# kasirershahartau/tissue_image_processing

Measured on AMD Instinct MI355X. Metric: frames/sec end-to-end (2048^2, z=30), higher is better.
Workload: dtype f32(f16x3)

## Files before the change

include/tissue_hip.h:

```cpp
#ifndef TISSUE_HIP_H
#define TISSUE_HIP_H

#include <stddef.h>
#include <stdint.h>

#ifdef __cplusplus
extern "C" {
#endif

#define TIP_API __attribute__((visibility("default")))

typedef enum {
    TIP_OK = 0,
    TIP_ERR_HIP = -1,
    TIP_ERR_ARG = -2,
    TIP_ERR_NOMEM = -3,
    TIP_ERR_INDEX = -4,
    TIP_ERR_UNSUPPORTED = -5,
    TIP_ERR_OVERFLOW = -6
} tip_status;

TIP_API int tip_init(int device);
TIP_API int tip_shutdown(void);
TIP_API int tip_last_error(char *buf, size_t n);
// ... 62 lines not shown
    const void *in0, *in1;
    int c0, c1, h, w, planes;
    const void *weights;
    int ntaps, dy[9], dx[9];
    int cout;
    const float *bias, *scale, *shift;
    void *out;
    int out_h, out_w, sy, sx, oy, ox;
    void *pool_out;
    const float *head_w, *head_b;
    float *head_out;
    int format;
    float acc_scale;
} tip_unet_conv_desc;
TIP_API int tip_unet_conv_dev(const tip_unet_conv_desc *d, void *stream);
TIP_API int tip_unet_conv_first_dev(const float *in, int h, int w, const float *wgt, const float *bias, const float *scale,
                                    const float *shift, void *out, int planes, int format, void *stream);
TIP_API int tip_unet_pool2_dev(const void *in, int h, int w, int ch, int planes, int format, void *out, void *stream);
TIP_API int tip_unet_head_dev(const void *in, long npix, const float *wgt, const float *bias, float *out, int planes, int format,
                              int logits, void *stream);
TIP_API int tip_unet_prepare_f64_dev(const double *img, int c, int a, int b, long cstride, long sa, long sb, int kind, float *out,
                                     int ap, int bp, void *stream);
TIP_API int tip_unet_tail_dev(const void *p, int dtype, long ld, int y, int x, double thr, int32_t *labels, double *hc,
                              int32_t *flags_host);

TIP_API int tip_draw_cell_types_u8(const uint8_t *types, long n, int must_mask, int lack_mask, const double *pos_rgb,
                                   const double *neg_rgb, double *out3);
TIP_API int tip_draw_tracking_i32(const int32_t *track, long n, const double *cycle18, double *out3);
TIP_API int tip_draw_disks_f64(int y, int x, int n, const double *cy, const double *cx, double radius, const double *rgb, double *out3);
TIP_API int tip_draw_lines_f64(int y, int x, int n, const int32_t *ends, const double *rgb, double *out3);
// ... 66 lines not shown
```

tissue_image_processing_amd/_unet_hip.py:

```python
import ctypes
import os
import threading

import numpy as np

from . import _lib

_MODES = {
    "f16x3": (2, 1, 3, "7.2e-7"),
    "bf16x3": (2, 0, 3, "1.6e-5"),
    "bf16x6": (3, 0, 6, "9e-8"),
}
_F16_ACT_SCALE = 16.0


class _ConvDesc(ctypes.Structure):
    _fields_ = [("in0", ctypes.c_void_p), ("in1", ctypes.c_void_p), ("c0", ctypes.c_int), ("c1", ctypes.c_int), ("h", ctypes.c_int),
                ("w", ctypes.c_int), ("planes", ctypes.c_int), ("weights", ctypes.c_void_p), ("ntaps", ctypes.c_int),
                ("dy", ctypes.c_int * 9), ("dx", ctypes.c_int * 9), ("cout", ctypes.c_int), ("bias", ctypes.c_void_p),
                ("scale", ctypes.c_void_p), ("shift", ctypes.c_void_p), ("out", ctypes.c_void_p), ("out_h", ctypes.c_int),
                ("out_w", ctypes.c_int), ("sy", ctypes.c_int), ("sx", ctypes.c_int), ("oy", ctypes.c_int), ("ox", ctypes.c_int),
                ("pool_out", ctypes.c_void_p), ("head_w", ctypes.c_void_p), ("head_b", ctypes.c_void_p), ("head_out", ctypes.c_void_p),
                ("format", ctypes.c_int), ("acc_scale", ctypes.c_float)]

# ... 151 lines not shown
        return out

    def first(h, w):
        out = buf(h, w, 128)
        timed("first %dx%d 2->128" % (h, w), 2.0 * h * w * 18 * 128,
              lambda: _lib.check(lib.tip_unet_conv_first_dev(D(x), h, w, D(hw["first"]), D(hw["f:d0.c1.b"]), D(hw["f:d0.b1.s"]),
                                                             D(hw["f:d0.b1.t"]), D(out), planes, fmt, stream)))
        return out

    def double(blk, src, skip, h, w, pooled=None, head=None):
        a = first(h, w) if src is None else conv3(blk + ".c1", blk + ".b1", src, skip, h, w)
        return conv3(blk + ".c2", blk + ".b2", a, None, h, w, pooled=pooled, head=head)

    def conv_t(name, src, h, w):
        up = buf(2 * h, 2 * w, hw[name + ".00"][0].shape[2] * 128)
        for py in (0, 1):
            for px in (0, 1):
                cls = "%s.%d%d" % (name, py, px)
                launch_conv(cls, _conv_desc(hw[cls], planes, fmt, src, None, h, w, hw["f:" + name + ".b"], out=up, out_h=2 * h, out_w=2 * w,
                                            stride=2, oy=py, ox=px))
        return up

    with torch.no_grad():
        skips, cur, h, w = [], None, H, W
        for i in range(3):
            pooled = buf(h // 2, w // 2, net.filters[i])
            skips.append(double("d%d" % i, cur, None, h, w, pooled=pooled))
            cur, h, w = pooled, h // 2, w // 2
        cur = double("mid", cur, None, h, w)
        for i in range(3):
            up = conv_t("u%d.t" % i, cur, h, w)
            h, w = 2 * h, 2 * w
            probs = None
            if i == 2 and not logits and not os.environ.get("TISSUE_HIP_UNET_SEPARATE_HEAD"):
                probs = torch.empty((1, 2, H, W), dtype=torch.float32, device=x.device)
# ... 9 lines not shown
```

tissue_image_processing_amd/csrc/tip_core.hip:

```cpp
#include "tip_internal.h"
#include <algorithm>
#include <cmath>
#include <cstdlib>
#include <map>
#include <mutex>

namespace tip {

static thread_local Ctx *g_ctx = nullptr;
static thread_local int g_requested_device = 0;

static int ctx_create(int device)
{
    Ctx *c = new Ctx();
    c->device = device;
    hipError_t e = hipSetDevice(device);
    if (e != hipSuccess) {
        c->err = std::string("hipSetDevice failed: ") + hipGetErrorString(e);
        g_ctx = c;
        return TIP_ERR_HIP;
    }
    {
        const char *pr = getenv("TIP_STREAM_PRIORITY");
        int lo = 0, hi = 0;
// ... 126 lines not shown
    }
    else if (n == "TIP_WS_OPEN") pair(t.ws_open_a, t.ws_open_b, def.ws_open_a, def.ws_open_b);
    else if (n == "TIP_WS_NO_SKIP") flag(t.ws_no_skip, 0);
    else if (n == "TIP_WS_DEBUG") flag(t.ws_debug, 0);
    else if (n == "TIP_WS_NO_ENDGAME") flag(t.ws_no_endgame, 0);
    else if (n == "TIP_WS_NO_WIDE") flag(t.ws_no_wide, 0);
    else if (n == "TIP_PROJECT_GENERIC") flag(t.project_generic, 0);
    else if (n == "TIP_PROJECT_UNFUSED_PREBLUR") flag(t.project_unfused_preblur, 0);
    else if (n == "TIP_PROJECT_UNFUSED_MASK") flag(t.project_unfused_mask, 0);
    else if (n == "TIP_PROJECT_EXACT_SCORE") flag(t.project_exact_score, 0);
    else if (n == "TIP_PROJECT_DEBUG") flag(t.project_debug, 0);
    else if (n == "TIP_UNET_TILE8") num(t.unet_tile8, def.unet_tile8);
    else if (n == "TIP_UF_ONE_LEVEL") flag(t.uf_one_level, 0);
    else if (n == "TIP_UNET_SPB") num(t.unet_spb, def.unet_spb);
    else if (n == "TIP_UNET_XCD_MAP") flag(t.unet_xcd_map, 1);
    else if (n == "TIP_UNET_TAIL_UNFUSED") flag(t.unet_tail_unfused, 0);
    else if (n == "TIP_MB_SMALL") num(t.mb_small, def.mb_small);
    else if (n == "TIP_MB_BATCH") num(t.mb_batch, def.mb_batch);
    else return false;
    return true;
}

const char *const TUNING_NAMES[] = {"TIP_WS_TIES", "TIP_WS_OPEN", "TIP_WS_NO_SKIP", "TIP_WS_DEBUG", "TIP_WS_NO_ENDGAME", "TIP_WS_NO_WIDE",
                                    "TIP_PROJECT_GENERIC", "TIP_PROJECT_UNFUSED_PREBLUR", "TIP_PROJECT_UNFUSED_MASK",
                                    "TIP_PROJECT_EXACT_SCORE", "TIP_PROJECT_DEBUG", "TIP_UNET_TILE8", "TIP_UNET_TAIL_UNFUSED", "TIP_UNET_XCD_MAP", "TIP_UNET_SPB", "TIP_UF_ONE_LEVEL", "TIP_MB_SMALL", "TIP_MB_BATCH"};

void tuning_from_env()
{
    for (const char *name : TUNING_NAMES)
        if (const char *e = getenv(name)) tuning_assign(g_tuning, name, e);
}
}

const Tuning &tuning()
{
    std::call_once(g_tuning_once, tuning_from_env);
    return g_tuning;
}

int make_taps(Taps &t, const double *w, int n)
// ... 225 lines not shown
```

tissue_image_processing_amd/csrc/tip_internal.h:

```cpp
#pragma once
#include <hip/hip_runtime.h>
#include <cstdarg>
#include <cstdint>
#include <cstdio>
#include <cstring>
#include <string>
#include <vector>
#include "../../include/tissue_hip.h"

namespace tip {

struct ProfRec { const char *name; hipEvent_t e0, e1; };

struct Ctx {
    int device = -1;
    hipStream_t stream = nullptr;
    std::string err;
    struct Block { void *p; size_t bytes; bool used; };
    std::vector<Block> pool;
    int last_ws_labels = 0;
    long last_ws_other = 0;
    hipEvent_t edge_event = nullptr;
    void *prep_ws = nullptr;
    void *pin_buf = nullptr;
// ... 20 lines not shown
};

void prof_begin(const char *name);
void prof_end();

struct Tuning {
    int ws_ties = 1;
    int ws_open_a = -1, ws_open_b = -1;
    int ws_no_skip = 0;
    int ws_debug = 0;
    int ws_no_endgame = 0, ws_no_wide = 0;
    int project_generic = 0, project_unfused_preblur = 0, project_unfused_mask = 0;
    int project_exact_score = 0, project_debug = 0;
    int unet_tail_unfused = 0;
    int unet_xcd_map = 1;
    int unet_spb = 3;
    int uf_one_level = 0;
    int mb_small = -1;
    int mb_batch = -1;
    int unet_tile8 = -1;
};
const Tuning &tuning();

#define TIP_HIP(call)                                                                             \
    do {                                                                                          \
        hipError_t e__ = (call);                                                                  \
        if (e__ != hipSuccess)                                                                    \
            return tip::fail(TIP_ERR_HIP, "%s failed: %s (%s:%d)", #call, hipGetErrorString(e__), \
                             __FILE__, __LINE__);                                                 \
    } while (0)
// ... 32 lines not shown
```

tissue_image_processing_amd/csrc/tip_unet.hip:

```cpp
#include "tip_internal.h"
#include "tip_unet_conv.h"
#include <algorithm>
#include <atomic>

namespace tip {

__global__ void __launch_bounds__(256) k_bias_relu_affine_f32(float *__restrict__ x, const float *__restrict__ bias,
                                                              const float *__restrict__ scale, const float *__restrict__ shift,
                                                              long n4, int C)
{
    const long i = (long)blockIdx.x * blockDim.x + threadIdx.x;
    if (i >= n4) return;
    float4 v = reinterpret_cast<float4 *>(x)[i];
    const int c = (int)((i * 4) % C);
    const float4 b = *reinterpret_cast<const float4 *>(bias + c);
    const float4 s = *reinterpret_cast<const float4 *>(scale + c);
    const float4 t = *reinterpret_cast<const float4 *>(shift + c);
    v.x += b.x; v.y += b.y; v.z += b.z; v.w += b.w;
    v.x = v.x > 0.f ? v.x : 0.f; v.y = v.y > 0.f ? v.y : 0.f; v.z = v.z > 0.f ? v.z : 0.f; v.w = v.w > 0.f ? v.w : 0.f;
    v.x = v.x * s.x + t.x; v.y = v.y * s.y + t.y; v.z = v.z * s.z + t.z; v.w = v.w * s.w + t.w;
    reinterpret_cast<float4 *>(x)[i] = v;
}

int rankfilter2d_dev(const void *in, void *out, int dtype, int Y, int X, int ky, int kx, int fp, int border, int is_max);
// ... 345 lines not shown
    for (int shift = 56; shift >= 0; shift -= 8) {
        hipLaunchKernelGGL(k_prep_hist, hgrid, dim3(256), 0, s, img, cstride, n, st, shift);
        hipLaunchKernelGGL(k_prep_pick, dim3(1), dim3(64), 0, s, st, c, shift);
    }
    hipLaunchKernelGGL(k_prep_next, hgrid, dim3(256), 0, s, img, cstride, n, st);
    hipLaunchKernelGGL(k_prep_finish, dim3(1), dim3(64), 0, s, st, c, g1, g99, kind);
    if (ap != a || bp != b) TIP_HIP(hipMemsetAsync(out, 0, (size_t)c * ap * bp * sizeof(float), s));
    const dim3 ngrid((unsigned)cdiv(a, 32), (unsigned)cdiv(b, 32), (unsigned)c);
    if (a_contig)
        hipLaunchKernelGGL(k_prep_normalize<true>, ngrid, dim3(256), 0, s, img, cstride, sa, sb, a, b, (const PrepState *)st, kind == 1 ? 1 : 0, out, ap, bp, ap - a, bp - b);
    else
        hipLaunchKernelGGL(k_prep_normalize<false>, ngrid, dim3(256), 0, s, img, cstride, sa, sb, a, b, (const PrepState *)st, kind == 1 ? 1 : 0, out, ap, bp, ap - a, bp - b);
    return unet_launch_check("unet_prepare");
}

int tip_unet_conv_dev(const tip_unet_conv_desc *d, void *stream)
{
    Ctx &c = ctx();
    if (!c.stream) return TIP_ERR_HIP;
    if (!d || !d->in0 || !d->weights || !d->bias || (!d->out && !d->head_out)) return fail(TIP_ERR_ARG, "tip_unet_conv_dev: null pointer");
    if (d->planes != 2 && d->planes != 3) return fail(TIP_ERR_ARG, "tip_unet_conv_dev: planes must be 2 or 3");
    if (d->format != 0 && d->format != 1) return fail(TIP_ERR_ARG, "tip_unet_conv_dev: format is 0 (bf16 pieces) or 1 (fp16 pieces)");
    if (d->format == 1 && (d->planes != 2 || !(d->acc_scale > 0.f))) return fail(TIP_ERR_ARG, "tip_unet_conv_dev: fp16 pieces come in two planes with a positive acc_scale");
    if (d->h < 8 || d->w < UC_TW || d->h % 8 || d->w % UC_TW)
        return fail(TIP_ERR_UNSUPPORTED, "tip_unet_conv_dev: the grid %dx%d is not a multiple of the 8x%d pixel tile", d->h, d->w, UC_TW);
    if (d->c0 < UC_KC || d->c0 % UC_KC || d->c1 < 0 || d->c1 % UC_KC || (d->c1 > 0 && !d->in1) || d->cout < UC_BN || d->cout % UC_BN)
        return fail(TIP_ERR_UNSUPPORTED, "tip_unet_conv_dev: channels (%d + %d -> %d) must be multiples of %d / %d", d->c0, d->c1, d->cout, UC_KC, UC_BN);
    if (d->ntaps < 1 || d->ntaps > 9 || d->sy < 1 || d->sx < 1 || d->oy < 0 || d->ox < 0 ||
        (d->h - 1) * d->sy + d->oy >= d->out_h || (d->w - 1) * d->sx + d->ox >= d->out_w)
        return fail(TIP_ERR_ARG, "tip_unet_conv_dev: bad taps / output mapping");
    if ((d->scale == nullptr) != (d->shift == nullptr)) return fail(TIP_ERR_ARG, "tip_unet_conv_dev: scale and shift come together");
    if (18L * d->w * (d->c0 > d->c1 ? d->c0 : d->c1) * 2 >= (1L << 32) - 65536)
        return fail(TIP_ERR_UNSUPPORTED, "tip_unet_conv_dev: 18 rows of %d pixels x %d channels exceed the 4 GB a buffer resource addresses",
                    d->w, d->c0 > d->c1 ? d->c0 : d->c1);
    ConvParams p;
    p.in0 = (const uint16_t *)d->in0; p.in1 = (const uint16_t *)(d->c1 > 0 ? d->in1 : d->in0);
    p.c0 = d->c0; p.c1 = d->c1; p.H = d->h; p.W = d->w;
    p.w = (const uint16_t *)d->weights; p.ntaps = d->ntaps;
    for (int t = 0; t < 9; ++t) {
        p.dy[t] = t < d->ntaps ? d->dy[t] : 0; p.dx[t] = t < d->ntaps ? d->dx[t] : 0;
        if (p.dy[t] < -1 || p.dy[t] > 1 || p.dx[t] < -1 || p.dx[t] > 1) return fail(TIP_ERR_ARG, "tip_unet_conv_dev: tap offsets are -1, 0 or 1");
    }
    p.cout = d->cout; p.bias = d->bias; p.scale = d->scale; p.shift = d->shift;
    p.out = (uint16_t *)d->out; p.outH = d->out_h; p.outW = d->out_w; p.sy = d->sy; p.sx = d->sx; p.oy = d->oy; p.ox = d->ox;
    p.pool_out = (uint16_t *)d->pool_out;
    p.acc_scale = d->format == 1 ? d->acc_scale : 1.f;
#ifdef UC_TRACE
    static unsigned long long *trace_dev = nullptr;
    if (!trace_dev) { TIP_HIP(hipMalloc(&trace_dev, 1024)); }
    TIP_HIP(hipMemsetAsync(trace_dev, 0, 1024, (hipStream_t)stream));
    p.trace = trace_dev;
#endif
    p.head_w = d->head_w; p.head_b = d->head_b; p.head_out = d->head_out;
    if (d->head_out && (!d->head_w || !d->head_b || d->cout != UC_BN || !d->scale || d->pool_out || d->sy != 1 || d->sx != 1 || d->oy != 0 || d->ox != 0 ||
                        d->out_h != d->h || d->out_w != d->w))
        return fail(TIP_ERR_ARG, "tip_unet_conv_dev: the fused head needs a 128-channel Conv2D + BatchNorm layer with the plain output mapping");
    if (d->pool_out && (d->sy != 1 || d->sx != 1 || d->oy != 0 || d->ox != 0 || d->out_h != d->h || d->out_w != d->w))
        return fail(TIP_ERR_ARG, "tip_unet_conv_dev: pool_out needs the plain output mapping");
    const int t8 = tuning().unet_tile8;
    const bool want8 = t8 == 1 || (t8 < 0 && d->ntaps == 9 && d->c0 + d->c1 <= 128);
    const int th = (d->planes == 2 && d->h % 16 == 0 && !want8) ? 16 : 8;
    const int dist = (th == 16 && d->ntaps >= 4) ? 4 : 2;
    const int da = (th == 16 && d->ntaps <= 2) ? 2 : 1;
    const int threads = th * 32, hp = UC_HW * (th + 2);
    const int ntiles = (d->h / th) * (d->w / UC_TW), nblks = d->cout / UC_BN;
    p.xcd_map = (tuning().unet_xcd_map && nblks > 1 && ntiles % 8 == 0) ? 1 : 0;
    const dim3 grid = p.xcd_map ? dim3((unsigned)(ntiles * nblks)) : dim3(ntiles, nblks);
    const int a_per = (d->planes * ((hp * 2 + 63) / 64) * 64 + threads - 1) / threads;
    const int spb = (th == 16 && dist == 4 && d->ntaps == 9 && tuning().unet_spb > 1) ? 3 : 1;
    const size_t lds = (size_t)(da + 1) * a_per * threads * 16 + (size_t)(spb > 1 ? 3 * spb : dist + 1) * d->planes * 256 * 16;
    hipStream_t s = (hipStream_t)stream;
    int which;
    if (d->planes == 3) which = 3;
    else if (th == 8) which = 0;
    else if (spb == 3) which = 6;
    else if (dist == 4) which = 2;
    else if (da == 2) which = 4;
    else which = 1;
    static std::atomic<unsigned> attr_done[64];
    const unsigned bit = 1u << (which + (d->format ? 9 : 0));
    const int dev = c.device >= 0 && c.device < 64 ? c.device : 0;
#define UC_FLAVOUR(W, ...)                                                                                                                  \
    case W: {                                                                                                                               \
        if (!(attr_done[dev].load(std::memory_order_acquire) & bit)) {                                                                      \
            TIP_HIP(hipFuncSetAttribute((const void *)(__VA_ARGS__), hipFuncAttributeMaxDynamicSharedMemorySize, (int)lds));                \
            attr_done[dev].fetch_or(bit, std::memory_order_release);                                                                        \
        }                                                                                                                                   \
        hipLaunchKernelGGL((__VA_ARGS__), grid, dim3(threads), lds, s, p);                                                                  \
    } break;
    if (d->format == 0) {
        switch (which) {
            UC_FLAVOUR(3, k_unet_conv<3, 8, 2>)
            UC_FLAVOUR(6, k_unet_conv<2, 16, 4, 1, 3>)
            UC_FLAVOUR(2, k_unet_conv<2, 16, 4>)
            UC_FLAVOUR(4, k_unet_conv<2, 16, 2, 2>)
            UC_FLAVOUR(1, k_unet_conv<2, 16, 2>)
            UC_FLAVOUR(0, k_unet_conv<2, 8, 2>)
        }
    } else {
        switch (which) {
            UC_FLAVOUR(6, k_unet_conv<2, 16, 4, 1, 3, true>)
            UC_FLAVOUR(2, k_unet_conv<2, 16, 4, 1, 1, true>)
            UC_FLAVOUR(4, k_unet_conv<2, 16, 2, 2, 1, true>)
            UC_FLAVOUR(1, k_unet_conv<2, 16, 2, 1, 1, true>)
            UC_FLAVOUR(0, k_unet_conv<2, 8, 2, 1, 1, true>)
// ... 5 lines not shown
        unsigned long long tr[128];
        TIP_HIP(hipStreamSynchronize(s));
        TIP_HIP(hipMemcpy(tr, trace_dev, sizeof tr, hipMemcpyDeviceToHost));
        for (int k = 0; k < th / 2; ++k) {
            const unsigned long long *t = tr + 16 * k;
            const double n = (double)t[4];
            fprintf(stderr, "UC_TRACE th %d spb %d taps %d cin %d cout %d grid %dx%d wave %d simd %d: per STEP (shader clocks; sums over the loop / steps): copies %.0f, products %.0f (first MFMA out after %.0f), "
                            "vmcnt wait %.0f, barrier %.0f, total %.0f; steps %.0f; whole loop %.0f, prologue %.0f, epilogue %.0f clocks\n",
                    th, spb, d->ntaps, d->c0 + d->c1, d->cout, d->h, d->w, k, (int)((t[7] >> 4) & 3), t[0] / n, t[2] / n, t[1] / n, t[6] / n, (t[3] - t[6]) / n, t[5] / n, n, (double)t[5], (double)t[8], (double)t[9]);
        }
    }
#endif
    return unet_launch_check("unet_conv");
}

int tip_unet_conv_first_dev(const float *in, int h, int w, const float *wgt, const float *bias, const float *scale, const float *shift,
                            void *out, int planes, int format, void *stream)
{
    Ctx &c = ctx();
    if (!c.stream) return TIP_ERR_HIP;
    if (!in || !wgt || !bias || !scale || !shift || !out || h < 1 || w < 1 || w % FIRST_RUN || ((long)h * w) % FIRST_PIX || (planes != 2 && planes != 3) ||
        (format != 0 && !(format == 1 && planes == 2)))
        return fail(TIP_ERR_ARG, "tip_unet_conv_first_dev: bad arguments (w must be a multiple of 32, h * w of 256)");
    const dim3 grid((unsigned)((long)h * w / FIRST_PIX));
    hipStream_t s = (hipStream_t)stream;
    if (format == 1) hipLaunchKernelGGL((k_unet_conv_first<2, true>), grid, dim3(256), 0, s, in, h, w, wgt, bias, scale, shift, (uint16_t *)out);
    else if (planes == 2) hipLaunchKernelGGL(k_unet_conv_first<2>, grid, dim3(256), 0, s, in, h, w, wgt, bias, scale, shift, (uint16_t *)out);
    else hipLaunchKernelGGL(k_unet_conv_first<3>, grid, dim3(256), 0, s, in, h, w, wgt, bias, scale, shift, (uint16_t *)out);
    return unet_launch_check("unet_conv_first");
}
// ... 31 lines not shown
```

tissue_image_processing_amd/csrc/tip_unet_conv.h:

```cpp
#pragma once
#include "tip_internal.h"

namespace tip {

typedef __bf16 bf16x8 __attribute__((ext_vector_type(8)));
typedef float f32x16 __attribute__((ext_vector_type(16)));
typedef __bf16 bf16x2 __attribute__((ext_vector_type(2)));
typedef float f32x2 __attribute__((ext_vector_type(2)));
typedef _Float16 f16x8 __attribute__((ext_vector_type(8)));
typedef _Float16 f16x2 __attribute__((ext_vector_type(2)));
constexpr float UC_F16_MAX = 65504.f;

constexpr int UC_TW = 32;
constexpr int UC_BN = 128;
constexpr int UC_KC = 16;
constexpr int UC_HW = UC_TW + 2;

struct ConvParams {
    const uint16_t *in0, *in1;
    int c0, c1;
    int H, W;
    const uint16_t *w;
    int ntaps;
    int dy[9], dx[9];
    int cout;
    const float *bias, *scale, *shift;
    uint16_t *out;
    int outH, outW, sy, sx, oy, ox;
    const float *head_w, *head_b;
    float *head_out;
#ifdef UC_TRACE
    unsigned long long *trace;
#endif
    int xcd_map;
    float acc_scale;
    uint16_t *pool_out;
};

__device__ __forceinline__ unsigned bf16_rne_bits(float v)
{
    const unsigned b = __float_as_uint(v);
    return (b + 0x7fffu + ((b >> 16) & 1u)) >> 16;
}
__device__ __forceinline__ float bf16_bits_to_f32(unsigned h) { return __uint_as_float(h << 16); }
__device__ __forceinline__ float relu_bits(float v) { return __int_as_float(max(__float_as_int(v), 0)); }
__device__ __forceinline__ float fmax_raw(float a, float b)
{
    float r;
    asm("v_max_f32 %0, %1, %2" : "=v"(r) : "v"(a), "v"(b));
    return r;
}
// ... 50 lines not shown
template <int N>
__device__ __forceinline__ unsigned long long uc_wait_barrier_timed()
{
    asm volatile("s_waitcnt vmcnt(%0) lgkmcnt(0)" ::"n"(N) : "memory");
    const unsigned long long t = __builtin_amdgcn_s_memtime();
    asm volatile("s_waitcnt lgkmcnt(0)\n\ts_barrier" ::: "memory");
    return t;
}
#endif
template <int N>
__device__ __forceinline__ void uc_wait_barrier()
{
    asm volatile("s_waitcnt vmcnt(%0) lgkmcnt(0)\n\ts_barrier" ::"n"(N) : "memory");
}

template <int NPL, int TH, int D, int DA = 1, int SPB = 1, bool F16 = false>
__global__ void __launch_bounds__(TH * 32, (NPL == 2) ? 2 : 1) k_unet_conv(const ConvParams p)
{
#if defined(__HIP_DEVICE_COMPILE__)
#ifdef UC_TRACE
    const unsigned long long tr_enter = __builtin_amdgcn_s_memtime();
#endif
    static_assert(DA == 1 || (DA == 2 && D == 2), "two-chunk activation prefetch: with the two-step weight schedule");
    static_assert(SPB == 1 || (SPB == 3 && D == 4 && DA == 1 && TH == 16), "several steps per barrier: the 16-row kernel with the four-step weight schedule");
    constexpr bool PAIR = SPB > 1;
    constexpr int UC_NBBUF = PAIR ? 3 * SPB : D + 1;
    constexpr int UC_THREADS = TH * 32, UC_HP = UC_HW * (TH + 2);
    static_assert(TH == 8 || (TH == 16 && NPL == 2), "16-row tiles: two pieces (LDS)");
    constexpr int A_GPP = (UC_HP * 2 + 63) / 64, A_PLANE = A_GPP * 64;
    constexpr int A_PER = (NPL * A_PLANE + UC_THREADS - 1) / UC_THREADS;
    constexpr int A_SLOTS = A_PER * UC_THREADS;
    constexpr int A_BYTES = A_SLOTS * 16;
    constexpr int B_PER = NPL * 256 / UC_THREADS;
    static_assert(B_PER * UC_THREADS == NPL * 256, "weight slots divide evenly");
    constexpr int B_BYTES = NPL * 256 * 16;
    extern __shared__ __attribute__((aligned(16))) unsigned char smem[];
    unsigned char *sA = smem, *sB = smem + (DA + 1) * A_BYTES;
    const int tid = threadIdx.x, lane = tid & 63;
    const int wave = __builtin_amdgcn_readfirstlane(tid >> 6);
    const int tilesX = p.W / UC_TW;
    const int nblks = p.cout / UC_BN;
    int tile, nblk;
    if (p.xcd_map) {
        const int b = blockIdx.x, xcd = b & 7, j = b >> 3;
        tile = (j / nblks) * 8 + xcd;
        nblk = j - (j / nblks) * nblks;
    } else {
        tile = blockIdx.x;
        nblk = blockIdx.y;
    }
    const int ty0 = (tile / tilesX) * TH, tx0 = (tile % tilesX) * UC_TW;
    const int cin = p.c0 + p.c1, nchunks = cin / UC_KC, nsteps = nchunks * p.ntaps;
    const long in_plane0 = (long)p.H * p.W * p.c0, in_plane1 = (long)p.H * p.W * p.c1;
    const int rowbase = ty0 > 0 ? ty0 - 1 : 0;
    const int winrows = min(p.H, ty0 + TH + 1) - rowbase;

    unsigned a_off[A_PER];
    auto plan_a = [&](int C) {
#pragma unroll
        for (int u = 0; u < A_PER; ++u) {
            const int g = u * (UC_THREADS / 64) + wave, pl = g / A_GPP;
            const int rem = (g - pl * A_GPP) * 64 + lane, px = rem >> 1, half = (rem & 1) ^ ((px >> 3) & 1);
            const int hy = px / UC_HW, hx = px - hy * UC_HW;
            const int gy = ty0 + hy - 1, gx = tx0 + hx - 1;
            const bool inside = pl < NPL && rem < UC_HP * 2 && gy >= 0 && gy < p.H && gx >= 0 && gx < p.W;
            a_off[u] = inside ? (unsigned)((((long)(gy - rowbase) * p.W + gx) * C + half * 8) * 2) : 0xffff0000u;
        }
    };
    plan_a(p.c0);
    bool a_second = false;
    constexpr int RSRC_FLAGS = 0x00020000;
    unsigned long long a_win = (unsigned long long)(p.in0 + (long)rowbase * p.W * p.c0), a_plane_bytes = (unsigned long long)in_plane0 * 2;
    int a_rec = (int)(unsigned)((long)winrows * p.W * p.c0 * 2);
    const __amdgpu_buffer_rsrc_t rs_b = __builtin_amdgcn_make_buffer_rsrc((void *)p.w, 0, (int)0xffffffffu, RSRC_FLAGS);
    auto copy_a = [&](int chunk, int buf) {
        const int cbase = chunk * UC_KC;
        const bool second = cbase >= p.c0;
        if (second && !a_second) {
            a_second = true;
            a_win = (unsigned long long)(p.in1 + (long)rowbase * p.W * p.c1);
            a_plane_bytes = (unsigned long long)in_plane1 * 2;
            a_rec = (int)(unsigned)((long)winrows * p.W * p.c1 * 2);
            if (p.c1 != p.c0) plan_a(p.c1);
        }
        const int soff = (second ? cbase - p.c0 : cbase) * 2;
        lds_byte *dst = (lds_byte *)(sA + buf * A_BYTES + wave * 64 * 16);
#pragma unroll
        for (int u = 0; u < A_PER; ++u) {
            const int pl = min((u * (UC_THREADS / 64) + wave) / A_GPP, NPL - 1);
// ... 11 lines not shown
#pragma unroll
        for (int u = 0; u < B_PER; ++u)
            __builtin_amdgcn_raw_ptr_buffer_load_lds(rs_b, dst + u * UC_THREADS * 16, 16, b_off, soff + u * (UC_THREADS / 256) * (UC_BN * UC_KC * 2), 0, 0);
    };

    f32x16 acc[2][4];
#pragma unroll
    for (int m = 0; m < 2; ++m)
#pragma unroll
        for (int n = 0; n < 4; ++n)
#pragma unroll
            for (int i = 0; i < 16; ++i) acc[m][n][i] = 0.f;

    copy_a(0, 0);
    if (DA == 2 && nchunks > 1) copy_a(1, 1);
    for (int s0 = 0; s0 < (PAIR ? 2 * SPB : D) && s0 < nsteps; ++s0) copy_b(s0 / p.ntaps, s0 % p.ntaps, s0);
    uc_wait_barrier<0>();

    const int r = lane & 31, h = lane >> 5;
    const int b_row = r * 2 + (h ^ ((r >> 3) & 1));
    int step = 0;
    int nc = D / p.ntaps, nt = D % p.ntaps;
    int buf0 = 0, buf2 = D;
    uint4 fa[2][NPL], fb[4][NPL];
#ifdef UC_TRACE
    unsigned long long tr_copy = 0, tr_read = 0, tr_mfma = 0, tr_bar = 0, tr_t0 = __builtin_amdgcn_s_memtime();
    const bool tracing = blockIdx.x == gridDim.x / 2 && blockIdx.y == 0;
    unsigned long long tr_wait = 0, t_w = 0;
#define UC_T(var) const unsigned long long var = __builtin_amdgcn_s_memtime()
#define UC_WB t_w = uc_wait_barrier_timed
#else
#define UC_T(var)
#define UC_WB uc_wait_barrier
#endif
#define UC_PRODUCT(PA, PB)                                                                                      \
    _Pragma("unroll") for (int m = 0; m < 2; ++m) _Pragma("unroll") for (int n = 0; n < 4; ++n)                 \
        acc[m][n] = uc_mfma<F16>(fb[n][PB], fa[m][PA], acc[m][n]);
    auto step_products = [&](int chunk, int tap) {
        const unsigned char *abuf = sA + (chunk % (DA + 1)) * A_BYTES;
        const unsigned char *bbuf = sB + buf0 * B_BYTES;
        const int dy = p.dy[tap], dx = p.dx[tap];
        int aslot[2];
#pragma unroll
        for (int m = 0; m < 2; ++m) {
            const int px = (wave * 2 + m + 1 + dy) * UC_HW + (r + 1 + dx);
            aslot[m] = px * 2 + (h ^ ((px >> 3) & 1));
        }
        auto read_a = [&](int m, int pl) { fa[m][pl] = *reinterpret_cast<const uint4 *>(abuf + (pl * A_PLANE + aslot[m]) * 16); };
        auto read_b = [&](int n, int pl) { fb[n][pl] = *reinterpret_cast<const uint4 *>(bbuf + (pl * 256 + n * 64 + b_row) * 16); };
        if constexpr (NPL == 2) {
            read_a(0, 1); read_a(1, 1);
#pragma unroll
            for (int n = 0; n < 4; ++n) read_b(n, 0);
            __builtin_amdgcn_sched_barrier(0);
            __builtin_amdgcn_s_setprio(1);
            acc[0][0] = uc_mfma<F16>(fb[0][0], fa[0][1], acc[0][0]);
// ... 18 lines not shown
#pragma unroll
                for (int m = 0; m < 2; ++m) read_a(m, NPL - 1 - k);
#pragma unroll
                for (int n = 0; n < 4; ++n) read_b(n, k);
            }
            __builtin_amdgcn_s_setprio(1);
            UC_PRODUCT(2, 0) UC_PRODUCT(1, 1) UC_PRODUCT(0, 2)
            UC_PRODUCT(1, 0)
            UC_PRODUCT(0, 1)
            UC_PRODUCT(0, 0)
            __builtin_amdgcn_s_setprio(0);
        }
    };
    if constexpr (PAIR) {
        int c0 = 0, t0 = 0;
        int cb = (2 * SPB) / p.ntaps, tb = (2 * SPB) % p.ntaps;
        int bb = 0;
        int a_issued = 0;
        auto next = [&](int &c, int &t) { if (++t == p.ntaps) { t = 0; ++c; } };
        auto wrapb = [](int b) { return b >= UC_NBBUF ? b - UC_NBBUF : b; };
        for (int s = 0; s < nsteps; s += SPB) {
            UC_T(t_a);
            const bool issue_a = c0 + 1 < nchunks && c0 + 1 > a_issued;
            const int ca = c0 + 1;
            if (issue_a) a_issued = ca;
            const bool issue_b = s + 2 * SPB < nsteps;
            UC_T(t_b);
#pragma unroll
            for (int k = 0; k < SPB; ++k) {
                buf0 = wrapb(bb + k);
                step_products(c0, t0);
                next(c0, t0);
                if (k == 0 && issue_a) copy_a(ca, ca & 1);
                if (issue_b) { copy_b(cb, tb, wrapb(bb + 2 * SPB + k)); next(cb, tb); }
            }
            UC_T(t_c);
            if (issue_b) { if (issue_a) UC_WB<A_PER + SPB * B_PER>(); else UC_WB<SPB * B_PER>(); }
            else { if (issue_a) UC_WB<A_PER>(); else UC_WB<0>(); }
            bb = wrapb(bb + SPB);
#ifdef UC_TRACE
            UC_T(t_d);
            tr_copy += t_b - t_a; tr_mfma += t_c - t_b; tr_bar += t_d - t_c; tr_wait += t_w - t_c;
#endif
        }
    } else
    for (int chunk = 0; chunk < nchunks; ++chunk) {
        for (int tap = 0; tap < p.ntaps; ++tap, ++step) {
            UC_T(t_a);
            const bool issue_a = tap == 0 && chunk + DA < nchunks;
            const bool issue_b = step + D < nsteps;
            UC_T(t_b);
            step_products(chunk, tap);
            if (issue_a) copy_a(chunk + DA, (chunk + DA) % (DA + 1));
            if (issue_b) copy_b(nc, nt, buf2);
            if (++nt == p.ntaps) { nt = 0; ++nc; }
            UC_T(t_c);
            if constexpr (D == 2) {
                const bool need_a_now = DA == 1 && issue_a && p.ntaps == 1;
                if (issue_b) {
                    if (issue_a && !need_a_now) UC_WB<A_PER + B_PER>(); else UC_WB<B_PER>();
                } else {
                    if (issue_a && !need_a_now) UC_WB<A_PER>(); else UC_WB<0>();
                }
            } else {
                const int left = nsteps - (step + 2);
                const int nb = left < 0 ? 0 : (left > D - 1 ? D - 1 : left);
                const bool a_out = tap <= D - 2 && chunk + 1 < nchunks;
#define UC_WAIT_CASE(NB_) case NB_: if (a_out) UC_WB<NB_ * B_PER + A_PER>(); else UC_WB<NB_ * B_PER>(); break;
                switch (nb) {
                    UC_WAIT_CASE(0) UC_WAIT_CASE(1) UC_WAIT_CASE(2)
                    default: if (a_out) UC_WB<(D - 1) * B_PER + A_PER>(); else UC_WB<(D - 1) * B_PER>(); break;
                }
#undef UC_WAIT_CASE
// ... 14 lines not shown
        tp[5] = __builtin_amdgcn_s_memtime() - tr_t0; tp[6] = tr_wait; tp[7] = (unsigned long long)__builtin_amdgcn_s_getreg((31 << 11) | 4);
        tp[8] = tr_t0 - tr_enter;
    }
    const unsigned long long tr_loop_end = __builtin_amdgcn_s_memtime();
#endif
#undef UC_PRODUCT

    constexpr int EP_ROW = 272, EP_BYTES = 32 * EP_ROW;
    static_assert(UC_THREADS / 64 * EP_BYTES <= (DA + 1) * A_BYTES + UC_NBBUF * B_BYTES, "the staging images fit the tile buffers");
    int pxl = lane & 31, hf = lane >> 5;
    asm volatile("" : "+v"(pxl), "+v"(hf));
    unsigned char *ep = smem + wave * EP_BYTES;
    {
        const float *bip = p.bias + nblk * UC_BN + 16 * hf;
        const float *scp = p.scale + nblk * UC_BN + 16 * hf, *shp = p.shift + nblk * UC_BN + 16 * hf;
        const f32x2 inv2 = {p.acc_scale, p.acc_scale};
        auto biased = [&](float a0, float a1, const f32x2 &b) -> f32x2 {
            if constexpr (F16) return __builtin_elementwise_fma(f32x2{a0, a1}, inv2, b);
            else return f32x2{a0, a1} + b;
        };
#pragma unroll
        for (int n = 0; n < 4; ++n) {
#pragma unroll
            for (int q = 0; q < 4; ++q) {
                const float4 b4 = *reinterpret_cast<const float4 *>(bip + n * 32 + q * 4);
                const f32x2 b01 = {b4.x, b4.y}, b23 = {b4.z, b4.w};
                if (p.scale) {
                    const float4 s4 = *reinterpret_cast<const float4 *>(scp + n * 32 + q * 4), t4 = *reinterpret_cast<const float4 *>(shp + n * 32 + q * 4);
                    const f32x2 s01 = {s4.x, s4.y}, s23 = {s4.z, s4.w}, t01 = {t4.x, t4.y}, t23 = {t4.z, t4.w};
#pragma unroll
                    for (int m = 0; m < 2; ++m) {
// ... 79 lines not shown
                w.y = piece_word(q8[n][2], q8[n][3], pl + 1 < NPL);
                w.z = piece_word(q8[n][4], q8[n][5], pl + 1 < NPL);
                w.w = piece_word(q8[n][6], q8[n][7], pl + 1 < NPL);
                *reinterpret_cast<uint4 *>(ep + (pxl >> 1) * EP_ROW + (n * 32 + 16 * hf + (oddp ? 8 : 0)) * 2) = w;
            }
#pragma unroll
            for (int it = 0; it < 4; ++it) {
                const int row = it * 4 + rd_row;
                *reinterpret_cast<uint4 *>(prow + pl * pool_plane + (long)row * p.cout) = *reinterpret_cast<const uint4 *>(ep + row * EP_ROW + rd_col);
            }
        }
    }
#pragma unroll
    for (int m = 0; m < 2; ++m) {
        const int y = ty0 + wave * 2 + m;
        uint16_t *orow = p.out + ((long)(y * p.sy + p.oy) * p.outW + ((long)tx0 * p.sx + p.ox)) * p.cout + nblk * UC_BN + (lane & 15) * 8;
#pragma unroll
        for (int pl = 0; pl < NPL; ++pl) {
#pragma unroll
            for (int n = 0; n < 4; ++n)
#pragma unroll
                for (int q = 0; q < 2; ++q) {
                    float v[8];
#pragma unroll
                    for (int j = 0; j < 8; ++j) v[j] = acc[m][n][q * 8 + j];
                    uint4 w;
                    w.x = piece_word(v[0], v[1], pl + 1 < NPL);
                    w.y = piece_word(v[2], v[3], pl + 1 < NPL);
                    w.z = piece_word(v[4], v[5], pl + 1 < NPL);
                    w.w = piece_word(v[6], v[7], pl + 1 < NPL);
                    if (pl + 1 < NPL) {
// ... 184 lines not shown
```

Baseline: 19.11.

## Group transposed-conv parity classes into one grouped kernel launch

The four stride-2 transposed-conv parity classes were launched as separate conv kernels. They now go through a new entry point that can fold several classes into one grid, with the class index taken from the block index, per-class weights, taps, offsets and acc_scale held in the params, and A-tile halo loads trimmed to the rows and columns the class's taps actually use. By default only classes with fewer than 4 taps are grouped, and the rest keep their own launches. This cuts launch count and fills the GPU better at the small decoder resolutions, at the cost of a uniform pipeline depth (dist 2, da 2) for the grouped flavour.

```diff
diff --git a/include/tissue_hip.h b/include/tissue_hip.h
--- a/include/tissue_hip.h
+++ b/include/tissue_hip.h
@@ -100,6 +100,7 @@
     float acc_scale;
 } tip_unet_conv_desc;
 TIP_API int tip_unet_conv_dev(const tip_unet_conv_desc *d, void *stream);
+TIP_API int tip_unet_convt_dev(const tip_unet_conv_desc *d, int n, void *stream);
 TIP_API int tip_unet_conv_first_dev(const float *in, int h, int w, const float *wgt, const float *bias, const float *scale,
                                     const float *shift, void *out, int planes, int format, void *stream);
 TIP_API int tip_unet_pool2_dev(const void *in, int h, int w, int ch, int planes, int format, void *out, void *stream);
diff --git a/tissue_image_processing_amd/_unet_hip.py b/tissue_image_processing_amd/_unet_hip.py
--- a/tissue_image_processing_amd/_unet_hip.py
+++ b/tissue_image_processing_amd/_unet_hip.py
@@ -189,11 +189,11 @@
 
     def conv_t(name, src, h, w):
         up = buf(2 * h, 2 * w, hw[name + ".00"][0].shape[2] * 128)
-        for py in (0, 1):
-            for px in (0, 1):
-                cls = "%s.%d%d" % (name, py, px)
-                launch_conv(cls, _conv_desc(hw[cls], planes, fmt, src, None, h, w, hw["f:" + name + ".b"], out=up, out_h=2 * h, out_w=2 * w,
-                                            stride=2, oy=py, ox=px))
+        ds = (_ConvDesc * 4)(*[_conv_desc(hw["%s.%d%d" % (name, py, px)], planes, fmt, src, None, h, w, hw["f:" + name + ".b"], out=up,
+                                          out_h=2 * h, out_w=2 * w, stride=2, oy=py, ox=px) for py in (0, 1) for px in (0, 1)])
+        d = ds[0]
+        timed("%s %dx%d %d+%d->%d x%d taps" % (name, d.h, d.w, d.c0, d.c1, d.cout, sum(e.ntaps for e in ds)),
+              2.0 * d.h * d.w * sum(e.ntaps for e in ds) * d.cout * (d.c0 + d.c1), lambda: _lib.check(lib.tip_unet_convt_dev(ds, 4, stream)))
         return up
 
     with torch.no_grad():
diff --git a/tissue_image_processing_amd/csrc/tip_core.hip b/tissue_image_processing_amd/csrc/tip_core.hip
--- a/tissue_image_processing_amd/csrc/tip_core.hip
+++ b/tissue_image_processing_amd/csrc/tip_core.hip
@@ -164,6 +164,7 @@
     else if (n == "TIP_UF_ONE_LEVEL") flag(t.uf_one_level, 0);
     else if (n == "TIP_UNET_SPB") num(t.unet_spb, def.unet_spb);
     else if (n == "TIP_UNET_XCD_MAP") flag(t.unet_xcd_map, 1);
+    else if (n == "TIP_UNET_CONVT_GROUP") num(t.unet_convt_group, def.unet_convt_group);
     else if (n == "TIP_UNET_TAIL_UNFUSED") flag(t.unet_tail_unfused, 0);
     else if (n == "TIP_MB_SMALL") num(t.mb_small, def.mb_small);
     else if (n == "TIP_MB_BATCH") num(t.mb_batch, def.mb_batch);
@@ -173,7 +174,7 @@
 
 const char *const TUNING_NAMES[] = {"TIP_WS_TIES", "TIP_WS_OPEN", "TIP_WS_NO_SKIP", "TIP_WS_DEBUG", "TIP_WS_NO_ENDGAME", "TIP_WS_NO_WIDE",
                                     "TIP_PROJECT_GENERIC", "TIP_PROJECT_UNFUSED_PREBLUR", "TIP_PROJECT_UNFUSED_MASK",
-                                    "TIP_PROJECT_EXACT_SCORE", "TIP_PROJECT_DEBUG", "TIP_UNET_TILE8", "TIP_UNET_TAIL_UNFUSED", "TIP_UNET_XCD_MAP", "TIP_UNET_SPB", "TIP_UF_ONE_LEVEL", "TIP_MB_SMALL", "TIP_MB_BATCH"};
+                                    "TIP_PROJECT_EXACT_SCORE", "TIP_PROJECT_DEBUG", "TIP_UNET_TILE8", "TIP_UNET_TAIL_UNFUSED", "TIP_UNET_XCD_MAP", "TIP_UNET_CONVT_GROUP", "TIP_UNET_SPB", "TIP_UF_ONE_LEVEL", "TIP_MB_SMALL", "TIP_MB_BATCH"};
 
 void tuning_from_env()
 {
diff --git a/tissue_image_processing_amd/csrc/tip_internal.h b/tissue_image_processing_amd/csrc/tip_internal.h
--- a/tissue_image_processing_amd/csrc/tip_internal.h
+++ b/tissue_image_processing_amd/csrc/tip_internal.h
@@ -58,6 +58,7 @@
     int project_exact_score = 0, project_debug = 0;
     int unet_tail_unfused = 0;
     int unet_xcd_map = 1;
+    int unet_convt_group = 3;
     int unet_spb = 3;
     int uf_one_level = 0;
     int mb_small = -1;
diff --git a/tissue_image_processing_amd/csrc/tip_unet.hip b/tissue_image_processing_amd/csrc/tip_unet.hip
--- a/tissue_image_processing_amd/csrc/tip_unet.hip
+++ b/tissue_image_processing_amd/csrc/tip_unet.hip
@@ -383,10 +383,11 @@
     return unet_launch_check("unet_prepare");
 }
 
-int tip_unet_conv_dev(const tip_unet_conv_desc *d, void *stream)
-{
-    Ctx &c = ctx();
-    if (!c.stream) return TIP_ERR_HIP;
+static int unet_conv_launch(const tip_unet_conv_desc *d, int ncls, void *stream)
+{
+    Ctx &c = ctx();
+    if (!c.stream) return TIP_ERR_HIP;
+    const bool grouped = ncls > 1;
     if (!d || !d->in0 || !d->weights || !d->bias || (!d->out && !d->head_out)) return fail(TIP_ERR_ARG, "tip_unet_conv_dev: null pointer");
     if (d->planes != 2 && d->planes != 3) return fail(TIP_ERR_ARG, "tip_unet_conv_dev: planes must be 2 or 3");
     if (d->format != 0 && d->format != 1) return fail(TIP_ERR_ARG, "tip_unet_conv_dev: format is 0 (bf16 pieces) or 1 (fp16 pieces)");
@@ -410,6 +411,19 @@
         p.dy[t] = t < d->ntaps ? d->dy[t] : 0; p.dx[t] = t < d->ntaps ? d->dx[t] : 0;
         if (p.dy[t] < -1 || p.dy[t] > 1 || p.dx[t] < -1 || p.dx[t] > 1) return fail(TIP_ERR_ARG, "tip_unet_conv_dev: tap offsets are -1, 0 or 1");
     }
+    p.g = ConvParams::Group{};
+    if (grouped) {
+        int order[UC_GMAX];
+        for (int k = 0; k < ncls; ++k) order[k] = k;
+        std::stable_sort(order, order + ncls, [&](int a, int b) { return d[a].ntaps > d[b].ntaps; });
+        p.g.ncls = ncls;
+        for (int k = 0; k < ncls; ++k) {
+            const tip_unet_conv_desc &e = d[order[k]];
+            p.g.w[k] = (const uint16_t *)e.weights; p.g.ntaps[k] = e.ntaps; p.g.oy[k] = e.oy; p.g.ox[k] = e.ox;
+            p.g.acc_scale[k] = e.format == 1 ? e.acc_scale : 1.f;
+            for (int t = 0; t < e.ntaps; ++t) { p.g.dy[k][t] = e.dy[t]; p.g.dx[k][t] = e.dx[t]; }
+        }
+    }
     p.cout = d->cout; p.bias = d->bias; p.scale = d->scale; p.shift = d->shift;
     p.out = (uint16_t *)d->out; p.outH = d->out_h; p.outW = d->out_w; p.sy = d->sy; p.sx = d->sx; p.oy = d->oy; p.ox = d->ox;
     p.pool_out = (uint16_t *)d->pool_out;
@@ -429,12 +443,13 @@
     const int t8 = tuning().unet_tile8;
     const bool want8 = t8 == 1 || (t8 < 0 && d->ntaps == 9 && d->c0 + d->c1 <= 128);
     const int th = (d->planes == 2 && d->h % 16 == 0 && !want8) ? 16 : 8;
-    const int dist = (th == 16 && d->ntaps >= 4) ? 4 : 2;
-    const int da = (th == 16 && d->ntaps <= 2) ? 2 : 1;
+    const int dist = (th == 16 && d->ntaps >= 4 && !grouped) ? 4 : 2;
+    const int da = (th == 16 && (d->ntaps <= 2 || grouped)) ? 2 : 1;
     const int threads = th * 32, hp = UC_HW * (th + 2);
     const int ntiles = (d->h / th) * (d->w / UC_TW), nblks = d->cout / UC_BN;
-    p.xcd_map = (tuning().unet_xcd_map && nblks > 1 && ntiles % 8 == 0) ? 1 : 0;
-    const dim3 grid = p.xcd_map ? dim3((unsigned)(ntiles * nblks)) : dim3(ntiles, nblks);
+    const int per = nblks * ncls;
+    p.xcd_map = (tuning().unet_xcd_map && per > 1 && ntiles % 8 == 0) ? 1 : 0;
+    const dim3 grid = p.xcd_map ? dim3((unsigned)(ntiles * per)) : dim3(ntiles, per);
     const int a_per = (d->planes * ((hp * 2 + 63) / 64) * 64 + threads - 1) / threads;
     const int spb = (th == 16 && dist == 4 && d->ntaps == 9 && tuning().unet_spb > 1) ? 3 : 1;
     const size_t lds = (size_t)(da + 1) * a_per * threads * 16 + (size_t)(spb > 1 ? 3 * spb : dist + 1) * d->planes * 256 * 16;
@@ -447,7 +462,8 @@
     else if (da == 2) which = 4;
     else which = 1;
     static std::atomic<unsigned> attr_done[64];
-    const unsigned bit = 1u << (which + (d->format ? 9 : 0));
+    const int gwhich = d->planes == 3 ? 0 : (th == 8 ? 1 : 2);
+    const unsigned bit = grouped ? 1u << (18 + gwhich + (d->format ? 3 : 0)) : 1u << (which + (d->format ? 9 : 0));
     const int dev = c.device >= 0 && c.device < 64 ? c.device : 0;
 #define UC_FLAVOUR(W, ...)                                                                                                                  \
     case W: {                                                                                                                               \
@@ -457,7 +473,18 @@
         }                                                                                                                                   \
         hipLaunchKernelGGL((__VA_ARGS__), grid, dim3(threads), lds, s, p);                                                                  \
     } break;
-    if (d->format == 0) {
+    if (grouped && d->format == 0) {
+        switch (gwhich) {
+            UC_FLAVOUR(0, k_unet_conv<3, 8, 2, 1, 1, false, true>)
+            UC_FLAVOUR(1, k_unet_conv<2, 8, 2, 1, 1, false, true>)
+            UC_FLAVOUR(2, k_unet_conv<2, 16, 2, 2, 1, false, true>)
+        }
+    } else if (grouped) {
+        switch (gwhich) {
+            UC_FLAVOUR(1, k_unet_conv<2, 8, 2, 1, 1, true, true>)
+            UC_FLAVOUR(2, k_unet_conv<2, 16, 2, 2, 1, true, true>)
+        }
+    } else if (d->format == 0) {
         switch (which) {
             UC_FLAVOUR(3, k_unet_conv<3, 8, 2>)
             UC_FLAVOUR(6, k_unet_conv<2, 16, 4, 1, 3>)
@@ -493,6 +520,37 @@
     return unet_launch_check("unet_conv");
 }
 
+int tip_unet_conv_dev(const tip_unet_conv_desc *d, void *stream) { return unet_conv_launch(d, 1, stream); }
+
+int tip_unet_convt_dev(const tip_unet_conv_desc *d, int n, void *stream)
+{
+    if (!d || n < 1 || n > UC_GMAX) return fail(TIP_ERR_ARG, "tip_unet_convt_dev: 1 .. %d classes", UC_GMAX);
+    for (int k = 0; k < n; ++k) {
+        const tip_unet_conv_desc &e = d[k];
+        if (e.in0 != d->in0 || e.in1 != d->in1 || e.c0 != d->c0 || e.c1 != d->c1 || e.h != d->h || e.w != d->w || e.planes != d->planes ||
+            e.format != d->format || e.cout != d->cout || e.bias != d->bias || e.scale != d->scale || e.shift != d->shift || e.out != d->out ||
+            e.out_h != d->out_h || e.out_w != d->out_w || e.sy != d->sy || e.sx != d->sx)
+            return fail(TIP_ERR_ARG, "tip_unet_convt_dev: the classes differ in more than weights, taps, output offset and acc_scale");
+        if (e.pool_out || e.head_out) return fail(TIP_ERR_ARG, "tip_unet_convt_dev: no pooled output, no fused head");
+        if (!e.weights || e.ntaps < 1 || e.ntaps > UC_GMAX) return fail(TIP_ERR_ARG, "tip_unet_convt_dev: a class has 1 .. %d taps", UC_GMAX);
+        if (e.oy < 0 || e.ox < 0 || (e.h - 1) * e.sy + e.oy >= e.out_h || (e.w - 1) * e.sx + e.ox >= e.out_w)
+            return fail(TIP_ERR_ARG, "tip_unet_convt_dev: bad output mapping");
+        if (e.format == 1 && !(e.acc_scale > 0.f)) return fail(TIP_ERR_ARG, "tip_unet_convt_dev: fp16 pieces need a positive acc_scale");
+        for (int t = 0; t < e.ntaps; ++t)
+            if (e.dy[t] < -1 || e.dy[t] > 1 || e.dx[t] < -1 || e.dx[t] > 1) return fail(TIP_ERR_ARG, "tip_unet_convt_dev: tap offsets are -1, 0 or 1");
+    }
+    const int mode = tuning().unet_convt_group;
+    tip_unet_conv_desc grp[UC_GMAX];
+    int ng = 0;
+    for (int k = 0; k < n; ++k) {
+        if (mode == 0 || (mode == 3 && d[k].ntaps >= 4)) {
+            if (int rc = unet_conv_launch(d + k, 1, stream)) return rc;
+        } else
+            grp[ng++] = d[k];
+    }
+    return ng ? unet_conv_launch(grp, ng, stream) : TIP_OK;
+}
+
 int tip_unet_conv_first_dev(const float *in, int h, int w, const float *wgt, const float *bias, const float *scale, const float *shift,
                             void *out, int planes, int format, void *stream)
 {
diff --git a/tissue_image_processing_amd/csrc/tip_unet_conv.h b/tissue_image_processing_amd/csrc/tip_unet_conv.h
--- a/tissue_image_processing_amd/csrc/tip_unet_conv.h
+++ b/tissue_image_processing_amd/csrc/tip_unet_conv.h
@@ -15,6 +15,7 @@
 constexpr int UC_BN = 128;
 constexpr int UC_KC = 16;
 constexpr int UC_HW = UC_TW + 2;
+constexpr int UC_GMAX = 4;
 
 struct ConvParams {
     const uint16_t *in0, *in1;
@@ -35,6 +36,12 @@
     int xcd_map;
     float acc_scale;
     uint16_t *pool_out;
+    struct Group {
+        int ncls;
+        const uint16_t *w[UC_GMAX];
+        int ntaps[UC_GMAX], dy[UC_GMAX][UC_GMAX], dx[UC_GMAX][UC_GMAX], oy[UC_GMAX], ox[UC_GMAX];
+        float acc_scale[UC_GMAX];
+    } g;
 };
 
 __device__ __forceinline__ unsigned bf16_rne_bits(float v)
@@ -115,7 +122,7 @@
     asm volatile("s_waitcnt vmcnt(%0) lgkmcnt(0)\n\ts_barrier" ::"n"(N) : "memory");
 }
 
-template <int NPL, int TH, int D, int DA = 1, int SPB = 1, bool F16 = false>
+template <int NPL, int TH, int D, int DA = 1, int SPB = 1, bool F16 = false, bool GRP = false>
 __global__ void __launch_bounds__(TH * 32, (NPL == 2) ? 2 : 1) k_unet_conv(const ConvParams p)
 {
 #if defined(__HIP_DEVICE_COMPILE__)
@@ -141,8 +148,21 @@
     const int wave = __builtin_amdgcn_readfirstlane(tid >> 6);
     const int tilesX = p.W / UC_TW;
     const int nblks = p.cout / UC_BN;
-    int tile, nblk;
-    if (p.xcd_map) {
+    int tile, nblk, cls = 0;
+    if constexpr (GRP) {
+        const int per = p.g.ncls * nblks;
+        int rem;
+        if (p.xcd_map) {
+            const int b = blockIdx.x, xcd = b & 7, j = b >> 3;
+            tile = (j / per) * 8 + xcd;
+            rem = j - (j / per) * per;
+        } else {
+            tile = blockIdx.x;
+            rem = blockIdx.y;
+        }
+        cls = rem / nblks;
+        nblk = rem - cls * nblks;
+    } else if (p.xcd_map) {
         const int b = blockIdx.x, xcd = b & 7, j = b >> 3;
         tile = (j / nblks) * 8 + xcd;
         nblk = j - (j / nblks) * nblks;
@@ -150,11 +170,21 @@
         tile = blockIdx.x;
         nblk = blockIdx.y;
     }
+    const int ntaps = GRP ? p.g.ntaps[cls] : p.ntaps;
     const int ty0 = (tile / tilesX) * TH, tx0 = (tile % tilesX) * UC_TW;
-    const int cin = p.c0 + p.c1, nchunks = cin / UC_KC, nsteps = nchunks * p.ntaps;
+    const int cin = p.c0 + p.c1, nchunks = cin / UC_KC, nsteps = nchunks * ntaps;
     const long in_plane0 = (long)p.H * p.W * p.c0, in_plane1 = (long)p.H * p.W * p.c1;
     const int rowbase = ty0 > 0 ? ty0 - 1 : 0;
     const int winrows = min(p.H, ty0 + TH + 1) - rowbase;
+    [[maybe_unused]] int hy0, hy1, hx0, hx1;
+    if constexpr (GRP) {
+        int dy0 = 1, dy1 = -1, dx0 = 1, dx1 = -1;
+        for (int t = 0; t < ntaps; ++t) {
+            dy0 = min(dy0, p.g.dy[cls][t]); dy1 = max(dy1, p.g.dy[cls][t]);
+            dx0 = min(dx0, p.g.dx[cls][t]); dx1 = max(dx1, p.g.dx[cls][t]);
+        }
+        hy0 = 1 + dy0; hy1 = TH + dy1; hx0 = 1 + dx0; hx1 = UC_TW + dx1;
+    }
 
     unsigned a_off[A_PER];
     auto plan_a = [&](int C) {
@@ -164,7 +194,8 @@
             const int rem = (g - pl * A_GPP) * 64 + lane, px = rem >> 1, half = (rem & 1) ^ ((px >> 3) & 1);
             const int hy = px / UC_HW, hx = px - hy * UC_HW;
             const int gy = ty0 + hy - 1, gx = tx0 + hx - 1;
-            const bool inside = pl < NPL && rem < UC_HP * 2 && gy >= 0 && gy < p.H && gx >= 0 && gx < p.W;
+            bool inside = pl < NPL && rem < UC_HP * 2 && gy >= 0 && gy < p.H && gx >= 0 && gx < p.W;
+            if constexpr (GRP) inside = inside && hy >= hy0 && hy <= hy1 && hx >= hx0 && hx <= hx1;
             a_off[u] = inside ? (unsigned)((((long)(gy - rowbase) * p.W + gx) * C + half * 8) * 2) : 0xffff0000u;
         }
     };
@@ -173,7 +204,7 @@
     constexpr int RSRC_FLAGS = 0x00020000;
     unsigned long long a_win = (unsigned long long)(p.in0 + (long)rowbase * p.W * p.c0), a_plane_bytes = (unsigned long long)in_plane0 * 2;
     int a_rec = (int)(unsigned)((long)winrows * p.W * p.c0 * 2);
-    const __amdgpu_buffer_rsrc_t rs_b = __builtin_amdgcn_make_buffer_rsrc((void *)p.w, 0, (int)0xffffffffu, RSRC_FLAGS);
+    const __amdgpu_buffer_rsrc_t rs_b = __builtin_amdgcn_make_buffer_rsrc((void *)(GRP ? p.g.w[cls] : p.w), 0, (int)0xffffffffu, RSRC_FLAGS);
     auto copy_a = [&](int chunk, int buf) {
         const int cbase = chunk * UC_KC;
         const bool second = cbase >= p.c0;
@@ -215,13 +246,13 @@
 
     copy_a(0, 0);
     if (DA == 2 && nchunks > 1) copy_a(1, 1);
-    for (int s0 = 0; s0 < (PAIR ? 2 * SPB : D) && s0 < nsteps; ++s0) copy_b(s0 / p.ntaps, s0 % p.ntaps, s0);
+    for (int s0 = 0; s0 < (PAIR ? 2 * SPB : D) && s0 < nsteps; ++s0) copy_b(s0 / ntaps, s0 % ntaps, s0);
     uc_wait_barrier<0>();
 
     const int r = lane & 31, h = lane >> 5;
     const int b_row = r * 2 + (h ^ ((r >> 3) & 1));
     int step = 0;
-    int nc = D / p.ntaps, nt = D % p.ntaps;
+    int nc = D / ntaps, nt = D % ntaps;
     int buf0 = 0, buf2 = D;
     uint4 fa[2][NPL], fb[4][NPL];
 #ifdef UC_TRACE
@@ -240,7 +271,7 @@
     auto step_products = [&](int chunk, int tap) {
         const unsigned char *abuf = sA + (chunk % (DA + 1)) * A_BYTES;
         const unsigned char *bbuf = sB + buf0 * B_BYTES;
-        const int dy = p.dy[tap], dx = p.dx[tap];
+        const int dy = GRP ? p.g.dy[cls][tap] : p.dy[tap], dx = GRP ? p.g.dx[cls][tap] : p.dx[tap];
         int aslot[2];
 #pragma unroll
         for (int m = 0; m < 2; ++m) {
@@ -289,10 +320,10 @@
     };
     if constexpr (PAIR) {
         int c0 = 0, t0 = 0;
-        int cb = (2 * SPB) / p.ntaps, tb = (2 * SPB) % p.ntaps;
+        int cb = (2 * SPB) / ntaps, tb = (2 * SPB) % ntaps;
         int bb = 0;
         int a_issued = 0;
-        auto next = [&](int &c, int &t) { if (++t == p.ntaps) { t = 0; ++c; } };
+        auto next = [&](int &c, int &t) { if (++t == ntaps) { t = 0; ++c; } };
         auto wrapb = [](int b) { return b >= UC_NBBUF ? b - UC_NBBUF : b; };
         for (int s = 0; s < nsteps; s += SPB) {
             UC_T(t_a);
@@ -320,7 +351,7 @@
         }
     } else
     for (int chunk = 0; chunk < nchunks; ++chunk) {
-        for (int tap = 0; tap < p.ntaps; ++tap, ++step) {
+        for (int tap = 0; tap < ntaps; ++tap, ++step) {
             UC_T(t_a);
             const bool issue_a = tap == 0 && chunk + DA < nchunks;
             const bool issue_b = step + D < nsteps;
@@ -328,10 +359,10 @@
             step_products(chunk, tap);
             if (issue_a) copy_a(chunk + DA, (chunk + DA) % (DA + 1));
             if (issue_b) copy_b(nc, nt, buf2);
-            if (++nt == p.ntaps) { nt = 0; ++nc; }
+            if (++nt == ntaps) { nt = 0; ++nc; }
             UC_T(t_c);
             if constexpr (D == 2) {
-                const bool need_a_now = DA == 1 && issue_a && p.ntaps == 1;
+                const bool need_a_now = DA == 1 && issue_a && ntaps == 1;
                 if (issue_b) {
                     if (issue_a && !need_a_now) UC_WB<A_PER + B_PER>(); else UC_WB<B_PER>();
                 } else {
@@ -376,7 +407,8 @@
     {
         const float *bip = p.bias + nblk * UC_BN + 16 * hf;
         const float *scp = p.scale + nblk * UC_BN + 16 * hf, *shp = p.shift + nblk * UC_BN + 16 * hf;
-        const f32x2 inv2 = {p.acc_scale, p.acc_scale};
+        const float acc_scale = GRP ? p.g.acc_scale[cls] : p.acc_scale;
+        const f32x2 inv2 = {acc_scale, acc_scale};
         auto biased = [&](float a0, float a1, const f32x2 &b) -> f32x2 {
             if constexpr (F16) return __builtin_elementwise_fma(f32x2{a0, a1}, inv2, b);
             else return f32x2{a0, a1} + b;
@@ -486,7 +518,7 @@
 #pragma unroll
     for (int m = 0; m < 2; ++m) {
         const int y = ty0 + wave * 2 + m;
-        uint16_t *orow = p.out + ((long)(y * p.sy + p.oy) * p.outW + ((long)tx0 * p.sx + p.ox)) * p.cout + nblk * UC_BN + (lane & 15) * 8;
+        uint16_t *orow = p.out + ((long)(y * p.sy + (GRP ? p.g.oy[cls] : p.oy)) * p.outW + ((long)tx0 * p.sx + (GRP ? p.g.ox[cls] : p.ox))) * p.cout + nblk * UC_BN + (lane & 15) * 8;
 #pragma unroll
         for (int pl = 0; pl < NPL; ++pl) {
 #pragma unroll
```

Result: no change. 19.08 (-0.1%).
